# bmwoolf/mini_parallel

Measured on AMD Instinct MI355X. Metric: GCUPS (billion cell updates/s) on 150bp reads, 1/2/4/8 MI355X; bit-exact scores, higher is better.
Workload: dtype f16

## Files before the change

mini_parallel_amd/csrc/msw_device.h:

```cpp
#pragma once
#include "msw_kernels.h"

#include <type_traits>

namespace msw {

typedef unsigned short u16x2 __attribute__((ext_vector_type(2)));
typedef _Float16 f16x2 __attribute__((ext_vector_type(2)));

__device__ __forceinline__ uint32_t pk_satsub(uint32_t a, uint32_t b) {
    return __builtin_bit_cast(uint32_t, __builtin_elementwise_sub_sat(
        __builtin_bit_cast(u16x2, a), __builtin_bit_cast(u16x2, b)));
}
__device__ __forceinline__ uint32_t pk_add(uint32_t a, uint32_t b) {
    return __builtin_bit_cast(uint32_t, __builtin_bit_cast(u16x2, a) + __builtin_bit_cast(u16x2, b));
}
__device__ __forceinline__ uint32_t pk_min(uint32_t a, uint32_t b) {
    return __builtin_bit_cast(uint32_t, __builtin_elementwise_min(
        __builtin_bit_cast(u16x2, a), __builtin_bit_cast(u16x2, b)));
}
__device__ __forceinline__ uint32_t pk_max(uint32_t a, uint32_t b) {
    return __builtin_bit_cast(uint32_t, __builtin_elementwise_max(
        __builtin_bit_cast(u16x2, a), __builtin_bit_cast(u16x2, b)));
}
__device__ __forceinline__ uint32_t pk_max3(uint32_t a, uint32_t b, uint32_t c) {
    f16x2 x = __builtin_bit_cast(f16x2, a), y = __builtin_bit_cast(f16x2, b),
          z = __builtin_bit_cast(f16x2, c);
    return __builtin_bit_cast(uint32_t,
                              __builtin_elementwise_maximum(x, __builtin_elementwise_maximum(y, z)));
}
__device__ __forceinline__ uint32_t hadd(uint32_t a, uint32_t b) {
    return __builtin_bit_cast(uint32_t, __builtin_bit_cast(f16x2, a) + __builtin_bit_cast(f16x2, b));
}
__device__ __forceinline__ uint32_t hadd_clamp(uint32_t a, uint32_t b) {
    const f16x2 z = {(_Float16)0.0f, (_Float16)0.0f}, one = {(_Float16)1.0f, (_Float16)1.0f};
    const f16x2 v = __builtin_bit_cast(f16x2, a) + __builtin_bit_cast(f16x2, b);
    return __builtin_bit_cast(uint32_t, __builtin_elementwise_min(__builtin_elementwise_max(v, z), one));
}
__device__ __forceinline__ uint32_t hmax(uint32_t a, uint32_t b) {
    return __builtin_bit_cast(uint32_t, __builtin_elementwise_maximum(__builtin_bit_cast(f16x2, a),
                                                                      __builtin_bit_cast(f16x2, b)));
}
__device__ __forceinline__ uint32_t f16_to_score(uint32_t bits) {
    return (uint32_t)((float)__builtin_bit_cast(_Float16, (unsigned short)bits) * 2048.0f);
}

__device__ __forceinline__ uint32_t track_max3(uint32_t best, uint32_t a, uint32_t b) {
    uint32_t d;
    asm("v_pk_maximum3_f16 %0, %1, %2, %3" : "=v"(d) : "v"(best), "v"(a), "v"(b));
    return d;
}

__device__ __forceinline__ uint32_t shr1_group(uint32_t src, uint32_t top_mask) {
    return (uint32_t)__builtin_amdgcn_update_dpp(0, (int)src, 0x138, 0xF, 0xF, true) & top_mask;
}

__device__ __forceinline__ uint32_t add_nc(uint32_t a, uint32_t b) { return a + b; }

__device__ __forceinline__ uint32_t hi_to_lo_own_lo_to_hi(uint32_t own, uint32_t dpp) {
    return __builtin_amdgcn_alignbit(own, dpp, 16);
}

struct PairMeta {
    uint32_t pa, pb;
    uint32_t oa, ob;
    bool va, vb;
    int ma, mb, na, nb;
    int64_t sa, sb;
};

#ifndef MSW_PROBE_NO_WIN
#define MSW_PROBE_NO_WIN 0
#endif
#ifndef MSW_PROBE_NO_READ
#define MSW_PROBE_NO_READ 0
#endif
#ifndef MSW_PROBE_CONST_LEN
#define MSW_PROBE_CONST_LEN 0
#endif

template <bool SPLIT, bool GEN>
__device__ __forceinline__ PairMeta load_meta(const SwParams& p, int g, uint32_t block, bool active) {
    PairMeta q;
    const uint32_t slot_a = block * pairs_per_wave(SPLIT, p.groups) + (SPLIT ? g : 2u * g);
    const uint32_t slot_b = SPLIT ? slot_a : slot_a + 1;
    const uint32_t last = p.n_slots - 1;
    const uint32_t sa = min(slot_a, last), sb = min(slot_b, last);
    q.va = active && slot_a < p.n_slots;
    q.vb = active && slot_b < p.n_slots;
    q.pa = p.order ? p.order[sa] : p.slot_base + sa;
    q.pb = SPLIT ? q.pa : (p.order ? p.order[sb] : p.slot_base + sb);
    q.oa = p.out_by_slot ? p.out_slot_base + sa : q.pa;
    q.ob = p.out_by_slot ? p.out_slot_base + sb : q.pb;
    int ma, na, mb, nb;
    if (p.slot_lens) {
        const uint32_t la = p.slot_lens[p.out_slot_base + sa];
        const uint32_t lb = SPLIT ? la : p.slot_lens[p.out_slot_base + sb];
        ma = (int)(la & 0xFFFFu);
        na = (int)(la >> 16);
        mb = (int)(lb & 0xFFFFu);
        nb = (int)(lb >> 16);
    } else if (MSW_PROBE_CONST_LEN) {
        ma = mb = 150;
        na = nb = 300;
    } else {
        ma = p.read_len[q.pa];
        na = p.win_len[q.pa];
        mb = SPLIT ? ma : (int)p.read_len[q.pb];
        nb = SPLIT ? na : (int)p.win_len[q.pb];
    }
    q.ma = q.va ? ma : 0;
    q.mb = q.vb ? mb : 0;
    q.na = q.va ? na : 0;
    q.nb = q.vb ? nb : 0;
    if constexpr (GEN) {
        const int64_t sa = p.win_pos[q.pa];
        const int64_t sb = SPLIT ? sa : p.win_pos[q.pb];
        q.sa = q.na > 0 ? sa : 0;
        q.sb = q.nb > 0 ? sb : 0;
    }
    return q;
}

template <bool GEN>
__device__ __forceinline__ const uint8_t* win_row(const SwParams& p, uint32_t pair, int64_t pos) {
    if constexpr (GEN) return p.win_src + pos;
    else return p.wins + (uint64_t)pair * p.win_stride;
}

template <bool GEN>
__device__ __forceinline__ uint4 win_chunk(const uint8_t* row, int k) {
    const uint8_t* a = row + 16 * k;
    if constexpr (!GEN) {
        return *reinterpret_cast<const uint4*>(a);
    } else {
        const uint32_t b = (uint32_t)(reinterpret_cast<uintptr_t>(a) & 3u);
        const uint32_t* al = reinterpret_cast<const uint32_t*>(a - b);
        const uint32_t x0 = al[0], x1 = al[1], x2 = al[2], x3 = al[3], x4 = al[4];
        return make_uint4(__builtin_amdgcn_alignbyte(x1, x0, b), __builtin_amdgcn_alignbyte(x2, x1, b),
                          __builtin_amdgcn_alignbyte(x3, x2, b), __builtin_amdgcn_alignbyte(x4, x3, b));
    }
}

template <bool GEN>
__device__ __forceinline__ int win_last(const SwParams& p, int n) {
    if constexpr (GEN) return max(n, 1) - 1;
    else return (int)p.win_stride - 1;
}

__device__ __forceinline__ int wave_max_i32(int v) {
#pragma unroll
    for (int off = 32; off > 0; off >>= 1) v = max(v, __shfl_xor(v, off, 64));
    return v;
}

__device__ __forceinline__ int wave_max_nonneg(int v) {
    v = max(v, __builtin_amdgcn_update_dpp(0, v, 0x111, 0xF, 0xF, true));
    v = max(v, __builtin_amdgcn_update_dpp(0, v, 0x112, 0xF, 0xF, true));
    v = max(v, __builtin_amdgcn_update_dpp(0, v, 0x114, 0xF, 0xF, true));
    v = max(v, __builtin_amdgcn_update_dpp(0, v, 0x118, 0xF, 0xF, true));
    v = max(v, __builtin_amdgcn_update_dpp(0, v, 0x142, 0xA, 0xF, false));
    v = max(v, __builtin_amdgcn_update_dpp(0, v, 0x143, 0xC, 0xF, false));
    return __builtin_amdgcn_readlane(v, 63);
}

__device__ __forceinline__ uint32_t wcode(uint32_t byte, bool valid, uint32_t shift) {
    return valid ? (byte << shift) : kWinSentinel;
}

template <bool SPLIT, bool GEN>
__device__ __forceinline__ void stage_window(const SwParams& p, const PairMeta& q, uint32_t* stream,
                                             int steps, int lg, int G, bool active) {
    if (!active) return;
    const uint8_t* wa = win_row<GEN>(p, q.pa, q.sa);
    const uint8_t* wb = win_row<GEN>(p, q.pb, q.sb);
    const uint32_t sh = p.code_shift;
    const int last = win_last<GEN>(p, q.na), last_b = win_last<GEN>(p, q.nb);
    for (int k = lg; k < kLead; k += G) stream[k] = kWinSentinel2;
    const int nch = (steps + 15) >> 4;
    if (p.win_vec) {
        const int loadable = (int)(p.win_stride >> 4);
        const int top_a = GEN ? max((q.na + 15) / 16 - 1, 0) : 0, top_b = GEN ? max((q.nb + 15) / 16 - 1, 0) : 0;
        for (int k0 = 0; k0 < nch; k0 += 2 * G) {
            uint4 va[2], vb[2];
            uint32_t prev[2];
#pragma unroll
            for (int u = 0; u < 2; ++u) {
                const int k = k0 + u * G + lg;
                if constexpr (GEN) {
                    va[u] = win_chunk<true>(wa, min(k, top_a));
                    if constexpr (SPLIT) prev[u] = wa[min(max(16 * k - 1, 0), last)];
                    else vb[u] = win_chunk<true>(wb, min(k, top_b));
                } else {
                    const bool ld = k < nch && k < loadable && !MSW_PROBE_NO_WIN;
                    va[u] = ld ? *reinterpret_cast<const uint4*>(wa + 16 * k) : make_uint4(0, 0, 0, 0);
                    if constexpr (SPLIT) {
                        prev[u] = wa[min(max(16 * k - 1, 0), last)];
                    } else {
                        vb[u] = ld ? *reinterpret_cast<const uint4*>(wb + 16 * k) : make_uint4(0, 0, 0, 0);
                    }
                }
            }
#pragma unroll
            for (int u = 0; u < 2; ++u) {
                const int k = k0 + u * G + lg;
                if (k < nch) {
                    const uint32_t xa[4] = {va[u].x, va[u].y, va[u].z, va[u].w};
                    uint32_t xb[4] = {0u, 0u, 0u, 0u};
                    if constexpr (!SPLIT) { xb[0] = vb[u].x; xb[1] = vb[u].y; xb[2] = vb[u].z; xb[3] = vb[u].w; }
                    uint4* dst = reinterpret_cast<uint4*>(stream + kLead + 16 * k);
                    uint32_t carry = 0u;
                    if constexpr (SPLIT) carry = prev[u] & 0xFFu;
#pragma unroll
                    for (int d = 0; d < 4; ++d) {
                        uint32_t w4[4];
#pragma unroll
                        for (int e = 0; e < 4; ++e) {
                            const int c = 16 * k + 4 * d + e;
                            const uint32_t ba = (xa[d] >> (8 * e)) & 0xFFu;
                            if constexpr (SPLIT) {
                                w4[e] = wcode(ba, c < q.na, sh) | (wcode(carry, c >= 1 && c - 1 < q.na, sh) << 16);
                                carry = ba;
                            } else {
                                const uint32_t bb = (xb[d] >> (8 * e)) & 0xFFu;
                                w4[e] = wcode(ba, c < q.na, sh) | (wcode(bb, c < q.nb, sh) << 16);
                            }
                        }
                        dst[d] = make_uint4(w4[0], w4[1], w4[2], w4[3]);
                    }
                }
            }
        }
    } else {
        for (int c0 = 0; c0 < steps; c0 += 4 * G) {
            uint32_t ba[4], bb[4];
#pragma unroll
            for (int u = 0; u < 4; ++u) {
                const int c = c0 + u * G + lg;
                ba[u] = wa[min(c, last)];
                bb[u] = SPLIT ? wa[min(max(c - 1, 0), last)] : wb[min(c, GEN ? last_b : last)];
            }
#pragma unroll
            for (int u = 0; u < 4; ++u) {
                const int c = c0 + u * G + lg;
                const bool vb = SPLIT ? (c >= 1 && c - 1 < q.na) : (c < q.nb);
                if (c < steps) stream[kLead + c] = wcode(ba[u], c < q.na, sh) | (wcode(bb[u], vb, sh) << 16);
            }
        }
    }
}

template <int KR, bool SPLIT>
__device__ __forceinline__ void load_read_bytes(const SwParams& p, uint32_t pa, uint32_t pb, int lg,
                                                uint32_t (&ba)[KR], uint32_t (&bb)[KR]) {
    const uint8_t* ra = p.reads + (uint64_t)pa * p.read_stride;
    const uint8_t* rb = p.reads + (uint64_t)pb * p.read_stride;
    const int last = (int)p.read_stride - 1;
#pragma unroll
    for (int r = 0; r < KR; ++r) {
        const int ia = SPLIT ? lg * 2 * KR + r : lg * KR + r;
        const int ib = SPLIT ? ia + KR : ia;
#if MSW_PROBE_NO_READ
        ba[r] = (uint32_t)(ia + pa) & 3u;
        bb[r] = (uint32_t)(ib + pb) & 3u;
        (void)ra; (void)rb; (void)last;
#else
        ba[r] = ra[min(ia, last)];
        bb[r] = rb[min(ib, last)];
#endif
    }
}

template <int KR, bool SPLIT>
__device__ __forceinline__ void read_codes(const SwParams& p, const PairMeta& q, int lg, const uint32_t (&ba)[KR],
                                           const uint32_t (&bb)[KR], uint32_t (&rc)[KR]) {
#pragma unroll
    for (int r = 0; r < KR; ++r) {
        const int ia = SPLIT ? lg * 2 * KR + r : lg * KR + r;
        const int ib = SPLIT ? ia + KR : ia;
        const uint32_t ca = ia < q.ma ? (ba[r] << p.code_shift) : kReadSentinel;
        const uint32_t cb = ib < q.mb ? (bb[r] << p.code_shift) : kReadSentinel;
        rc[r] = ca | (cb << 16);
    }
}

__device__ __forceinline__ uint32_t group_pk_max(uint32_t v, int lg, int G) {
    const int lane = threadIdx.x;
#pragma unroll
    for (int off = 1; off < 16; off <<= 1) {
        const uint32_t o = (uint32_t)__shfl((int)v, lane + off, 64);
        v = lg + off < G ? pk_max(v, o) : v;
    }
    return v;
}

__device__ __forceinline__ uint64_t group_max_u64(uint64_t v, int lg, int G) {
    const int lane = threadIdx.x;
#pragma unroll
    for (int off = 1; off < 16; off <<= 1) {
        const uint64_t o = __shfl(v, lane + off, 64);
        v = (lg + off < G && o > v) ? o : v;
    }
    return v;
}

__device__ __forceinline__ void store_score(const SwParams& p, bool valid, uint32_t pair, uint32_t s) {
    if (valid) p.score[pair] = (int32_t)s;
}

__device__ __forceinline__ void store_hit(const SwParams& p, bool valid, uint32_t pair, uint64_t key,
                                          uint32_t bias, bool f16) {
    if (!valid) return;
    const uint32_t s = f16 ? f16_to_score((uint32_t)(key >> 32)) : (uint32_t)(key >> 32) - bias;
    p.score[pair] = (int32_t)s;
    if (p.end_i) {
        const uint32_t lo = (uint32_t)key;
        p.end_i[pair] = s ? (int16_t)(0xFFFFu - (lo >> 16)) : (int16_t)-1;
        p.end_j[pair] = s ? (int16_t)(0xFFFFu - (lo & 0xFFFFu)) : (int16_t)-1;
    }
}

template <int KR, bool SPLIT>
__device__ __forceinline__ void finish_coords(const SwParams& p, const PairMeta& q, int lg, int G,
                                              const uint32_t (&key_a)[KR], const uint32_t (&key_b)[KR],
                                              uint32_t bias, bool f16) {
    uint64_t ga = 0, gb = 0;
#pragma unroll
    for (int r = 0; r < KR; ++r) {
        const uint32_t ia = SPLIT ? (uint32_t)(lg * 2 * KR + r) : (uint32_t)(lg * KR + r);
        const uint32_t ib = SPLIT ? ia + KR : ia;
        const uint64_t ka = ((uint64_t)(key_a[r] >> 16) << 32) | ((uint64_t)(0xFFFFu - ia) << 16) |
                            (key_a[r] & 0xFFFFu);
        const uint64_t kb = ((uint64_t)(key_b[r] >> 16) << 32) | ((uint64_t)(0xFFFFu - ib) << 16) |
                            (key_b[r] & 0xFFFFu);
        ga = ka > ga ? ka : ga;
        gb = kb > gb ? kb : gb;
    }
    if constexpr (SPLIT) {
        ga = gb > ga ? gb : ga;
        ga = group_max_u64(ga, lg, G);
        if (lg == 0) store_hit(p, q.va, q.oa, ga, bias, f16);
    } else {
        ga = group_max_u64(ga, lg, G);
        gb = group_max_u64(gb, lg, G);
        if (lg == 0) {
            store_hit(p, q.va, q.oa, ga, bias, f16);
            store_hit(p, q.vb, q.ob, gb, bias, f16);
        }
    }
}

template <bool SPLIT>
__device__ __forceinline__ void finish_score(const SwParams& p, const PairMeta& q, int lg, int G,
                                             uint32_t best, uint32_t bias, bool f16) {
    best = group_pk_max(best, lg, G);
    if (lg == 0) {
        auto val = [&](uint32_t h) { return f16 ? f16_to_score(h) : h - bias; };
        if constexpr (SPLIT) {
            store_score(p, q.va, q.oa, val(max(best & 0xFFFFu, best >> 16)));
        } else {
            store_score(p, q.va, q.oa, val(best & 0xFFFFu));
            store_score(p, q.vb, q.ob, val(best >> 16));
        }
    }
}

template <bool SPLIT>
__device__ __forceinline__ uint32_t from_above(uint32_t own_bottom, uint32_t top_mask) {
    const uint32_t d = shr1_group(own_bottom, top_mask);
    if constexpr (SPLIT) return hi_to_lo_own_lo_to_hi(own_bottom, d);
    else return d;
}

__device__ __forceinline__ uint32_t base_class(uint32_t b) { return ((b >> 1) ^ (b >> 2)) & 3u; }

__device__ __forceinline__ bool is_acgt(uint32_t b) {
    const uint32_t o = b - 0x41u;
    return o < 20u && ((0x80045u >> o) & 1u);
}

__device__ __forceinline__ bool code_ok(uint32_t v, uint32_t shift) {
    return (v & kWinSentinel) || is_acgt(v >> shift);
}

__device__ __forceinline__ uint32_t win_selector(uint32_t word, uint32_t shift) {
    const uint32_t lo = word & 0xFFFFu, hi = word >> 16;
    const uint32_t sl = (lo & kWinSentinel) ? 12u : base_class(lo >> shift);
    const uint32_t sh = (hi & kWinSentinel) ? 12u : 4u + base_class(hi >> shift);
    return 12u | (sl << 8) | (12u << 16) | (sh << 24);
}

__device__ __forceinline__ uint32_t row_table(uint32_t v, uint32_t shift, uint32_t mis4, uint32_t match_hi) {
    const uint32_t b = v >> shift;
    if ((v & kReadSentinel) || !is_acgt(b)) return mis4;
    const uint32_t sh = 8u * base_class(b);
    return (mis4 & ~(0xFFu << sh)) | (match_hi << sh);
}

__device__ __forceinline__ bool to_fast_path(uint32_t* stream, int words, int lg, int G, bool active,
                                             uint32_t shift, bool allowed) {
    if (!allowed) return false;
    bool ok = true;
    for (int k = lg; active && k < words; k += G) {
        const uint32_t w = stream[k];
        ok = ok && code_ok(w & 0xFFFFu, shift) && code_ok(w >> 16, shift);
    }
    if (__builtin_amdgcn_ballot_w64(!ok) != 0) return false;
    for (int k = lg; active && k < words; k += G) stream[k] = win_selector(stream[k], shift);
    __syncthreads();
    return true;
}

__device__ __forceinline__ uint32_t class4(uint32_t x) { return ((x >> 1) ^ (x >> 2)) & 0x03030303u; }
__device__ __forceinline__ uint32_t canon4(uint32_t cl) { return __builtin_amdgcn_perm(0u, 0x54474341u, cl); }
__device__ __forceinline__ uint32_t byte_mask(int rem) {
    return rem >= 4 ? ~0u : (rem <= 0 ? 0u : ~0u >> (32 - 8 * rem));
}

constexpr int kRound = 2;
struct WinRound {
    uint4 a[kRound], b[kRound];
    uint32_t prev[kRound];
};

template <bool SPLIT, bool GEN>
__device__ __forceinline__ void load_round(const SwParams& p, const PairMeta& q, int k0, int lg, int G,
                                           WinRound& w) {
    const uint8_t* wa = win_row<GEN>(p, q.pa, q.sa);
    const uint8_t* wb = win_row<GEN>(p, q.pb, q.sb);
    const int stream_top = (int)((p.lds_stride - kLead) >> 4);
    const int top = (GEN ? stream_top : min((int)(p.win_stride >> 4), stream_top)) - 1;
    const int top_a = max(min(top, ((q.na + 15) >> 4) - 1), 0);
    const int top_b = max(min(top, ((q.nb + 15) >> 4) - 1), 0);
    const int last = win_last<GEN>(p, q.na);
#pragma unroll
    for (int u = 0; u < kRound; ++u) {
        const int k = k0 + u * G + lg;
#if MSW_PROBE_NO_WIN
        w.a[u] = w.b[u] = make_uint4(0x03020100u + min(k, top), 0x01000302u, 0x02010003u, 0x00030201u ^ q.pa);
        w.prev[u] = 0;
        (void)wa; (void)wb; (void)last; (void)top_a; (void)top_b;
#else
        w.a[u] = win_chunk<GEN>(wa, min(k, top_a));
        if constexpr (SPLIT) w.prev[u] = wa[min(max(16 * k - 1, 0), last)];
        else w.b[u] = win_chunk<GEN>(wb, min(k, top_b));
#endif
    }
}

template <bool SPLIT>
__device__ __forceinline__ uint32_t sel_round(const PairMeta& q, uint32_t* stream, int k0, int nch, int lg, int G,
                                              const WinRound& w) {
    uint32_t bad = 0u;
#pragma unroll
    for (int u = 0; u < kRound; ++u) {
        const int k = k0 + u * G + lg;
        if (k < nch) {
            const uint32_t xa[4] = {w.a[u].x, w.a[u].y, w.a[u].z, w.a[u].w};
            uint32_t xb[4] = {0u, 0u, 0u, 0u};
            if constexpr (!SPLIT) { xb[0] = w.b[u].x; xb[1] = w.b[u].y; xb[2] = w.b[u].z; xb[3] = w.b[u].w; }
            uint32_t carry = SPLIT ? (w.prev[u] & 0xFFu) : 0u;
            uint4* dst = reinterpret_cast<uint4*>(stream + kLead + 16 * k);
#pragma unroll
            for (int d = 0; d < 4; ++d) {
                const int c0 = 16 * k + 4 * d;
                const uint32_t x_a = xa[d];
                const uint32_t ma = byte_mask(q.na - c0);
                uint32_t x_b, mb;
                if constexpr (SPLIT) {
                    x_b = (x_a << 8) | carry;
                    carry = x_a >> 24;
                    mb = byte_mask(q.na + 1 - c0) & (c0 == 0 ? ~0xFFu : ~0u);
                } else {
                    x_b = xb[d];
                    mb = byte_mask(q.nb - c0);
                }
                const uint32_t ca = class4(x_a), cb = class4(x_b);
                bad |= ((canon4(ca) ^ x_a) & ma) | ((canon4(cb) ^ x_b) & mb);
                const uint32_t sa = (ca & ma) | (0x0C0C0C0Cu & ~ma);
                const uint32_t sb = ((cb | 0x04040404u) & mb) | (0x0C0C0C0Cu & ~mb);
                uint32_t o[4];
#pragma unroll
                for (int e = 0; e < 4; ++e)
                    o[e] = __builtin_amdgcn_perm(sb, sa, 0x000C000Cu | (uint32_t)e << 8 | (uint32_t)(4 + e) << 24) |
                           0x000C000Cu;
                dst[d] = make_uint4(o[0], o[1], o[2], o[3]);
            }
        }
    }
    return bad;
}

constexpr bool explicit_sched(bool affine, bool coords) { return !affine || coords; }
constexpr int step_unroll(bool , bool coords) { return coords ? 2 : 4; }
constexpr int perm_lead(bool affine, bool coords) { return !affine && !coords ? 2 : 0; }

template <int KR, bool AFFINE, bool COORDS, bool SPLIT, bool GEN = false>
__device__ __forceinline__ bool sw_body(const SwParams& p, uint32_t block, uint32_t* lds, uint64_t& t_loop) {
    const int lane = threadIdx.x;
    const int G = (int)p.group_lanes;
    const int g_raw = lane / G;
    const bool active = g_raw < (int)p.groups;
    const int g = active ? g_raw : 0;
    const int lg = active ? lane - g_raw * G : 0;
    uint32_t top_mask = lg == 0 ? 0u : ~0u;
    asm volatile("" : "+v"(top_mask));
    const PairMeta q = load_meta<SPLIT, GEN>(p, g, block, active);
    uint32_t rb_a[KR], rb_b[KR];
    load_read_bytes<KR, SPLIT>(p, q.pa, q.pb, lg, rb_a, rb_b);
    const bool try_fast = p.f16_ok && p.win_vec;
    WinRound w0;
    if (try_fast) load_round<SPLIT, GEN>(p, q, 0, lg, G, w0);
    const int skew = SPLIT ? 2 * (G - 1) + 1 : G - 1;
    constexpr int kUnroll = (!SPLIT && explicit_sched(AFFINE, COORDS)) ? 4 : step_unroll(AFFINE, COORDS);
    const int steps = (wave_max_nonneg(max(q.na, q.nb)) + skew + kUnroll - 1) & ~(kUnroll - 1);
    uint32_t* stream = lds + g * p.lds_stride;
    uint32_t rc[KR];
    read_codes<KR, SPLIT>(p, q, lg, rb_a, rb_b, rc);
    bool fast;
    if (try_fast) {
        const int nch = (int)((p.lds_stride - kLead) >> 4);
        uint32_t bad = 0u;
        if (active) {
            for (int k = lg; k < kLead; k += G) stream[k] = 0x0C0C0C0Cu;
            bad = sel_round<SPLIT>(q, stream, 0, nch, lg, G, w0);
            for (int k0 = kRound * G; k0 < nch; k0 += kRound * G) {
                WinRound w;
                load_round<SPLIT, GEN>(p, q, k0, lg, G, w);
                bad |= sel_round<SPLIT>(q, stream, k0, nch, lg, G, w);
            }
        }
        fast = __builtin_amdgcn_ballot_w64(bad != 0u) == 0;
        if (!fast) stage_window<SPLIT, GEN>(p, q, stream, steps, lg, G, active);
    } else {
        stage_window<SPLIT, GEN>(p, q, stream, steps, lg, G, active);
        __syncthreads();
        fast = to_fast_path(stream, kLead + steps, lg, G, active, p.code_shift, p.f16_ok != 0);
    }
    __syncthreads();

    uint32_t E[KR], GK[AFFINE ? KR : 1];
    uint32_t key_a[COORDS ? KR : 1], key_b[COORDS ? KR : 1];
    uint32_t best = 0u;
    const uint32_t* wp = stream + (kLead - (SPLIT ? 2 * lg : lg));
    const uint32_t nj_lane = (uint32_t)(0xFFFF + (SPLIT ? 2 * lg : lg));
    const uint32_t lds_wp = (uint32_t)(uintptr_t)wp;

    auto run = [&](auto f16_tag) __attribute__((always_inline)) {
        constexpr bool F16 = decltype(f16_tag)::value;
        const uint32_t match2 = p.match2, delta2 = p.delta2, ext2 = p.gap2, oe2 = p.open_ext2;
        const uint32_t bias2 = (AFFINE && !F16) ? p.bias2 : 0u;
        const uint32_t kmatch2 = add_nc(bias2, match2);
        const uint32_t og2 = oe2 - bias2;
        const uint32_t nge = p.f16_ngap2, noe = p.f16_noe2;
        uint32_t tab_lo[F16 ? KR : 1], tab_hi[F16 ? KR : 1];
        if constexpr (F16) {
            const uint32_t mis4 = (p.f16_hi >> 8) * 0x01010101u, match_hi = p.f16_hi & 0xFFu;
#pragma unroll
            for (int r = 0; r < KR; ++r) {
                tab_lo[r] = row_table(rc[r] & 0xFFFFu, p.code_shift, mis4, match_hi);
                tab_hi[r] = row_table(rc[r] >> 16, p.code_shift, mis4, match_hi);
            }
        }
        auto sub = [&](int r, uint32_t w) __attribute__((always_inline)) -> uint32_t {
            if constexpr (F16) return __builtin_amdgcn_perm(tab_hi[r], tab_lo[r], w);
            else return pk_min(rc[r] ^ w, delta2);
        };
#pragma unroll
        for (int r = 0; r < KR; ++r) {
            E[r] = bias2;
            if constexpr (AFFINE) GK[r] = bias2;
            if constexpr (COORDS) { key_a[r] = 0u; key_b[r] = 0u; }
        }
        uint32_t f_bot = bias2, h_bot = bias2;

        uint32_t t1a[KR], t1b[KR];
        using P0 = std::integral_constant<int, 0>;
        using P1 = std::integral_constant<int, 1>;
        if constexpr (F16 && !SPLIT && explicit_sched(AFFINE, COORDS)) {
#define MSW_SB __builtin_amdgcn_sched_barrier(0)
            {
                const uint32_t w0 = wp[0];
#pragma unroll
                for (int r = 0; r < KR; ++r) t1a[r] = sub(r, w0);
            }
            uint32_t an0 = sub(0, wp[1]);
            uint32_t hpend = 0u, hkm2 = 0u;
            uint32_t hu = shr1_group(h_bot, top_mask);
            uint32_t fu = AFFINE ? shr1_group(f_bot, top_mask) : 0u;
            auto sstep = [&](int t, uint32_t w1, uint32_t w2, const uint32_t (&t1)[KR], uint32_t (&t1n)[KR],
                             auto parity) __attribute__((always_inline)) {
                constexpr int kParity = decltype(parity)::value;
                uint32_t up = 0u, g_up = 0u, e_next = 0u, fsub = 0u;
                if constexpr (AFFINE) {
                    fsub = hadd(fu, nge);
                    MSW_SB;
                    g_up = hadd_clamp(hu, noe);
                    MSW_SB;
                    const uint32_t el = hadd(E[0], nge);
                    MSW_SB;
                    t1n[0] = hadd(hu, an0);
                    MSW_SB;
                    e_next = hmax(el, GK[0]);
                    MSW_SB;
                } else {
                    up = hadd_clamp(hu, nge);
                    MSW_SB;
                    t1n[0] = hadd(hu, an0);
                    MSW_SB;
                }
                uint32_t nja = 0u;
                if constexpr (COORDS) {
                    nja = (nj_lane - (uint32_t)t) & 0xFFFFu;
                    MSW_SB;
                } else if constexpr (KR & 1) {
                    if constexpr (kParity == 0) {
                        best = track_max3(best, hpend, h_bot);
                        MSW_SB;
                    } else {
                        hpend = h_bot;
                    }
                } else {
                    best = track_max3(best, hkm2, h_bot);
                    MSW_SB;
                }
                uint32_t hh[KR];
                uint32_t ka = 0u, kb = 0u;
                auto key_form = [&](int r) __attribute__((always_inline)) {
                    ka = (hh[r] << 16) | nja;
                    MSW_SB;
                    kb = (hh[r] & 0xFFFF0000u) | nja;
                    MSW_SB;
                };
                auto key_fold = [&](int r) __attribute__((always_inline)) {
                    key_a[r] = max(key_a[r], ka);
                    MSW_SB;
                    key_b[r] = max(key_b[r], kb);
                    MSW_SB;
                };
#pragma unroll
                for (int r = 0; r < KR; ++r) {
                    const bool last = r + 1 == KR;
                    uint32_t h, a = 0u;
                    if constexpr (AFFINE) {
                        const uint32_t e = e_next;
                        const uint32_t F = hmax(fsub, g_up);
                        MSW_SB;
                        uint32_t el = 0u;
                        if (!last) {
                            el = hadd(E[r + 1], nge);
                            MSW_SB;
                            a = sub(r + 1, w1);
                        } else {
                            an0 = sub(0, w2);
                        }
                        MSW_SB;
                        h = pk_max3(t1[r], e, F);
                        MSW_SB;
                        hh[r] = h;
                        E[r] = e;
                        if (!last) fsub = hadd(F, nge);
                        else fu = shr1_group(F, top_mask);
                        MSW_SB;
                        if (!last) {
                            e_next = hmax(el, GK[r + 1]);
                            MSW_SB;
                        }
                        if constexpr (COORDS) {
                            if (r > 0) key_form(r - 1);
                        }
                        g_up = GK[r] = hadd_clamp(h, noe);
                        MSW_SB;
                    } else {
                        h = pk_max3(t1[r], E[r], up);
                        MSW_SB;
                        hh[r] = h;
                        if (!last) a = sub(r + 1, w1);
                        else an0 = sub(0, w2);
                        MSW_SB;
                        if constexpr (COORDS) {
                            if (r > 0) key_form(r - 1);
                        }
                        up = E[r] = hadd_clamp(h, nge);
                        MSW_SB;
                    }
                    if (!last) {
                        t1n[r + 1] = hadd(h, a);
                        MSW_SB;
                    }
                    if constexpr (COORDS) {
                        if (r > 0) key_fold(r - 1);
                    } else if (r >= 2 && (r & 1) == 0) {
                        best = track_max3(best, hh[r - 2], hh[r - 1]);
                        MSW_SB;
                    }
                }
                if constexpr (COORDS) {
                    key_form(KR - 1);
                    key_fold(KR - 1);
                }
                h_bot = hh[KR - 1];
                if constexpr (!COORDS && (KR & 1) == 0) hkm2 = hh[KR - 2];
                hu = shr1_group(h_bot, top_mask);
                MSW_SB;
            };
            uint2 wa = make_uint2(wp[1], wp[2]);
            uint2 wb;
            asm volatile("ds_read2_b32 %0, %1 offset0:3 offset1:4" : "=v"(wb) : "v"(lds_wp));
            for (int t = 0; t < steps; t += 4) {
                const uint32_t base = lds_wp + 4u * (uint32_t)t;
                asm volatile("s_waitcnt lgkmcnt(0)" : "+v"(wb));
                sstep(t, wa.x, wa.y, t1a, t1b, P0{});
                sstep(t + 1, wa.y, wb.x, t1b, t1a, P1{});
                asm volatile("ds_read2_b32 %0, %1 offset0:5 offset1:6" : "=v"(wa) : "v"(base));
                sstep(t + 2, wb.x, wb.y, t1a, t1b, P0{});
                asm volatile("s_waitcnt lgkmcnt(0)" : "+v"(wa));
                sstep(t + 3, wb.y, wa.x, t1b, t1a, P1{});
                asm volatile("ds_read2_b32 %0, %1 offset0:7 offset1:8" : "=v"(wb) : "v"(base));
            }
            asm volatile("s_waitcnt lgkmcnt(0)" : "+v"(wb));
            if constexpr (!COORDS) best = track_max3(best, (KR & 1) ? hpend : hkm2, h_bot);
#undef MSW_SB
            return;
        }
        {
            const uint32_t w0 = wp[0];
#pragma unroll
            for (int r = 0; r < KR; ++r) {
                const uint32_t a = sub(r, w0);
                t1a[r] = F16 ? a : (AFFINE ? kmatch2 - a : pk_satsub(match2, a));
            }
        }
        uint32_t hpend = 0u;
        auto step = [&](int t, uint32_t w, const uint32_t (&t1)[KR], uint32_t (&t1n)[KR], auto parity)
                        __attribute__((always_inline)) {
            constexpr int kParity = decltype(parity)::value;
            const uint32_t h_up = from_above<SPLIT>(h_bot - bias2, top_mask);
            uint32_t up;
            uint32_t g_up;
            if constexpr (F16) {
                if constexpr (AFFINE) {
                    up = from_above<SPLIT>(f_bot, top_mask);
                    g_up = hadd_clamp(h_up, noe);
                } else {
                    up = hadd_clamp(h_up, nge);
                    g_up = 0u;
                }
            } else if constexpr (AFFINE) {
                up = add_nc(from_above<SPLIT>(f_bot - bias2, top_mask), bias2);
                g_up = add_nc(pk_satsub(h_up, og2), bias2);
            } else {
                up = pk_satsub(h_up, ext2);
                g_up = 0u;
            }
            constexpr int kPermLead = F16 ? perm_lead(AFFINE, COORDS) : 0;
            uint32_t a_n[KR];
#pragma unroll
            for (int r = 0; r < KR; ++r)
                if (!kPermLead || r < kPermLead) a_n[r] = sub(r, w);
            if constexpr (F16) t1n[0] = hadd(h_up, a_n[0]);
            else t1n[0] = AFFINE ? add_nc(h_up, kmatch2) - a_n[0] : pk_satsub(add_nc(h_up, kmatch2), a_n[0]);
            const uint32_t nj_a = (nj_lane - (uint32_t)t) & 0xFFFFu;
            const uint32_t nj_b = SPLIT ? ((nj_lane + 1u - (uint32_t)t) & 0xFFFFu) : nj_a;
            uint32_t hprev = 0u;
#pragma unroll
            for (int r = 0; r < KR; ++r) {
                uint32_t h;
                if constexpr (F16) {
                    if (kPermLead && r + kPermLead < KR) a_n[r + kPermLead] = sub(r + kPermLead, w);
                    if constexpr (AFFINE) {
                        const uint32_t e = hmax(hadd(E[r], nge), GK[r]);
                        up = hmax(hadd(up, nge), g_up);
                        h = pk_max3(t1[r], e, up);
                        E[r] = e;
                        g_up = GK[r] = hadd_clamp(h, noe);
                    } else {
                        h = pk_max3(t1[r], E[r], up);
                        up = E[r] = hadd_clamp(h, nge);
                    }
                    if (r + 1 < KR) t1n[r + 1] = hadd(h, a_n[r + 1]);
                } else if constexpr (AFFINE) {
                    const uint32_t e = pk_max(E[r] - ext2, GK[r]);
                    up = pk_max(up - ext2, g_up);
                    h = pk_max3(t1[r], e, up);
                    E[r] = e;
                    g_up = GK[r] = add_nc(pk_satsub(h, oe2), bias2);
                    if (r + 1 < KR) t1n[r + 1] = add_nc(h, match2) - a_n[r + 1];
                } else {
                    h = pk_max3(t1[r], E[r], up);
                    up = E[r] = pk_satsub(h, ext2);
                    if (r + 1 < KR) t1n[r + 1] = pk_satsub(add_nc(h, match2), a_n[r + 1]);
                }
                if (r + 1 == KR) h_bot = h;
                if constexpr (COORDS) {
                    key_a[r] = max(key_a[r], (h << 16) | nj_a);
                    key_b[r] = max(key_b[r], (h & 0xFFFF0000u) | nj_b);
                } else {
                    if (r & 1) {
                        best = track_max3(best, hprev, h);
                    } else if (r + 1 == KR) {
                        if constexpr (kParity == 0) hpend = h;
                        else best = track_max3(best, hpend, h);
                    }
                    hprev = h;
                }
                if constexpr (kPermLead > 0) __builtin_amdgcn_sched_barrier(0);
            }
            if constexpr (AFFINE) f_bot = up;
        };
        if constexpr (kUnroll == 4) {
            uint2 wa = make_uint2(wp[1], wp[2]);
            uint2 wb;
            asm volatile("ds_read2_b32 %0, %1 offset0:3 offset1:4" : "=v"(wb) : "v"(lds_wp));
            for (int t = 0; t < steps; t += 4) {
                const uint32_t base = lds_wp + 4u * (uint32_t)t;
                step(t, wa.x, t1a, t1b, P0{});
                step(t + 1, wa.y, t1b, t1a, P1{});
                asm volatile("ds_read2_b32 %0, %1 offset0:5 offset1:6" : "=v"(wa) : "v"(base));
                asm volatile("s_waitcnt lgkmcnt(1)" : "+v"(wb));
                step(t + 2, wb.x, t1a, t1b, P0{});
                step(t + 3, wb.y, t1b, t1a, P1{});
                asm volatile("ds_read2_b32 %0, %1 offset0:7 offset1:8" : "=v"(wb) : "v"(base));
                asm volatile("s_waitcnt lgkmcnt(1)" : "+v"(wa));
            }
            asm volatile("s_waitcnt lgkmcnt(0)" : "+v"(wb));
        } else {
            uint32_t w1 = wp[1], w2 = wp[2];
            uint2 wn;
            asm volatile("ds_read2_b32 %0, %1 offset0:3 offset1:4" : "=v"(wn) : "v"(lds_wp));
            for (int t = 0; t < steps; t += 2) {
                step(t, w1, t1a, t1b, P0{});
                step(t + 1, w2, t1b, t1a, P1{});
                asm volatile("s_waitcnt lgkmcnt(0)" : "+v"(wn));
                w1 = wn.x;
                w2 = wn.y;
                asm volatile("ds_read2_b32 %0, %1 offset0:3 offset1:4"
                             : "=v"(wn) : "v"(lds_wp + 4u * (uint32_t)(t + 2)));
            }
            asm volatile("s_waitcnt lgkmcnt(0)" : "+v"(wn));
        }
    };
    if (p.trace) t_loop = __builtin_amdgcn_s_memrealtime();
    if (fast) run(std::true_type{});
    else run(std::false_type{});

    const uint32_t bias = fast ? 0u : (p.bias2 & 0xFFFFu) * (AFFINE ? 1u : 0u);
    if constexpr (COORDS) finish_coords<KR, SPLIT>(p, q, lg, G, key_a, key_b, bias, fast);
    else finish_score<SPLIT>(p, q, lg, G, best, bias, fast);
    return fast;
}

struct WaveClock {
    uint64_t t0, c0;
};
__device__ __forceinline__ WaveClock trace_begin(const SwParams& p) {
    WaveClock w{0, 0};
    if (p.trace) {
        w.t0 = __builtin_amdgcn_s_memrealtime();
        w.c0 = __builtin_amdgcn_s_memtime();
    }
    return w;
}
__device__ __forceinline__ void trace_end(const SwParams& p, const WaveClock& w, bool fast, bool split,
                                          int kr, uint64_t t_loop) {
    if (!p.trace) return;
    const uint64_t t1 = __builtin_amdgcn_s_memrealtime();
    const uint64_t c1 = __builtin_amdgcn_s_memtime();
    if (threadIdx.x == 0) {
        const uint32_t hw_id = __builtin_amdgcn_s_getreg((4) | (0 << 6) | (31 << 11));
        const uint32_t xcc = __builtin_amdgcn_s_getreg((20) | (0 << 6) | (3 << 11));
        uint64_t* o = p.trace + 4ull * blockIdx.x;
        o[0] = w.t0;
        o[1] = t1;
        o[2] = (uint64_t)hw_id | ((uint64_t)xcc << 32) | ((uint64_t)fast << 40) | ((uint64_t)split << 41) |
               ((uint64_t)kr << 48);
        o[3] = ((c1 - w.c0) & 0xFFFFFFFFFFull) | ((t_loop - w.t0) << 40);
    }
}

template <uint32_t G>
__device__ __forceinline__ uint32_t xcd_block(uint32_t b, uint32_t nb) {
    constexpr uint32_t span = 8u * G;
    const uint32_t base = b - b % span;
    if (base + span > nb) return b;
    const uint32_t r = b - base;
    return base + (r % 8u) * G + r / 8u;
}

template <int KR, bool AFFINE, bool COORDS, bool SPLIT, bool GEN = false>
__global__ __launch_bounds__(64) void sw_kernel(SwParams p) {
    extern __shared__ __attribute__((aligned(16))) uint32_t lds[];
    const WaveClock wc = trace_begin(p);
    uint64_t t_loop = 0;
    const bool fast = sw_body<KR, AFFINE, COORDS, SPLIT, GEN>(p, blockIdx.x, lds, t_loop);
    trace_end(p, wc, fast, SPLIT, KR, t_loop);
}

template <int KRP, bool AFFINE, bool COORDS>
__global__ __launch_bounds__(64) void sw_mixed_kernel(SwParams p) {
    extern __shared__ __attribute__((aligned(16))) uint32_t lds[];
    const WaveClock wc = trace_begin(p);
    uint64_t t_loop = 0;
    if (blockIdx.x < p.pairs_blocks) {
        const bool fast = sw_body<KRP, AFFINE, COORDS, false>(p, blockIdx.x, lds, t_loop);
        trace_end(p, wc, fast, false, KRP, t_loop);
    } else {
        SwParams q = p;
        const uint32_t done = p.pairs_blocks * pairs_per_wave(false, p.groups);
        q.n_slots = p.n_slots - done;
        q.order = p.order ? p.order + done : nullptr;
        if (!p.order) q.slot_base = done;
        q.out_slot_base = p.out_slot_base + done;
        const bool fast = sw_body<(KRP + 1) / 2, AFFINE, COORDS, true>(q, blockIdx.x - p.pairs_blocks, lds,
                                                                      t_loop);
        trace_end(p, wc, fast, true, (KRP + 1) / 2, t_loop);
    }
}

template <int KR, bool AFFINE, bool COORDS>
__device__ __forceinline__ void multi_body(const SwParams& q, uint32_t blk, uint32_t* lds) {
    const WaveClock wc = trace_begin(q);
    uint64_t t_loop = 0;
    const bool fast = sw_body<KR, AFFINE, COORDS, false>(q, blk, lds, t_loop);
    trace_end(q, wc, fast, false, KR, t_loop);
}

template <bool AFFINE, bool COORDS, bool WIDE = false>
__global__ __launch_bounds__(64) void sw_multi_kernel(SwParams p, MultiTable t) {
    extern __shared__ __attribute__((aligned(16))) uint32_t lds[];
    const uint32_t lb = xcd_block<4>(blockIdx.x, gridDim.x);
    uint32_t b = 0;
    while (b + 1 < t.n_buckets && lb >= t.block_end[b]) ++b;
    const uint32_t blk = lb - (b ? t.block_end[b - 1] : 0u);
    SwParams q = p;
    q.order = p.order + t.slot_begin[b];
    q.out_slot_base = p.out_slot_base + t.slot_begin[b];
    q.n_slots = t.count[b];
    q.lds_stride = t.lds_stride[b];
    q.f16_ok = t.f16_ok[b];
    if constexpr (WIDE) {
        switch (t.kr[b]) {
            case 17: multi_body<17, AFFINE, COORDS>(q, blk, lds); break;
            case 18: multi_body<18, AFFINE, COORDS>(q, blk, lds); break;
            case 19: multi_body<19, AFFINE, COORDS>(q, blk, lds); break;
            case 20: multi_body<20, AFFINE, COORDS>(q, blk, lds); break;
            case 21: multi_body<21, AFFINE, COORDS>(q, blk, lds); break;
            case 22: multi_body<22, AFFINE, COORDS>(q, blk, lds); break;
            case 23: multi_body<23, AFFINE, COORDS>(q, blk, lds); break;
            default: multi_body<24, AFFINE, COORDS>(q, blk, lds); break;
        }
    } else {
        switch (t.kr[b]) {
            case 1: multi_body<1, AFFINE, COORDS>(q, blk, lds); break;
            case 2: multi_body<2, AFFINE, COORDS>(q, blk, lds); break;
            case 3: multi_body<3, AFFINE, COORDS>(q, blk, lds); break;
            case 4: multi_body<4, AFFINE, COORDS>(q, blk, lds); break;
            case 5: multi_body<5, AFFINE, COORDS>(q, blk, lds); break;
            case 6: multi_body<6, AFFINE, COORDS>(q, blk, lds); break;
            case 7: multi_body<7, AFFINE, COORDS>(q, blk, lds); break;
            case 8: multi_body<8, AFFINE, COORDS>(q, blk, lds); break;
            case 9: multi_body<9, AFFINE, COORDS>(q, blk, lds); break;
            case 10: multi_body<10, AFFINE, COORDS>(q, blk, lds); break;
            case 11: multi_body<11, AFFINE, COORDS>(q, blk, lds); break;
            case 12: multi_body<12, AFFINE, COORDS>(q, blk, lds); break;
            case 13: multi_body<13, AFFINE, COORDS>(q, blk, lds); break;
            case 14: multi_body<14, AFFINE, COORDS>(q, blk, lds); break;
            case 15: multi_body<15, AFFINE, COORDS>(q, blk, lds); break;
            default: multi_body<16, AFFINE, COORDS>(q, blk, lds); break;
        }
    }
}

}
```

Baseline: 10570.

## Specialize prologue for identity order, pin kernel args, simplify f16 row tables

Adds an identity-order specialization of load_meta that skips the order and slot_lens indirect loads when both are null, and hoists metadata masking after the read and window loads are issued so memory latency overlaps. It pins all kernel arguments into SGPRs with an empty asm, and computes f16 substitution tables directly from raw read bytes with a branchless XOR trick instead of going through read_codes. Window chunk clamping by length is dropped on the non-planned, non-generated path. The aim is a shorter per-wave prologue, at the cost of more code paths and possible out-of-range window chunk reads when clamping is skipped.

```diff
diff --git a/mini_parallel_amd/csrc/msw_device.h b/mini_parallel_amd/csrc/msw_device.h
--- a/mini_parallel_amd/csrc/msw_device.h
+++ b/mini_parallel_amd/csrc/msw_device.h
@@ -79,7 +79,28 @@
 #define MSW_PROBE_CONST_LEN 0
 #endif
 
-template <bool SPLIT, bool GEN>
+__device__ __forceinline__ void pin_args(const SwParams& p) {
+    asm volatile("" ::"s"(p.reads), "s"(p.wins), "s"(p.read_len), "s"(p.win_len), "s"(p.order), "s"(p.slot_lens),
+                 "s"(p.read_stride), "s"(p.win_stride), "s"(p.n_slots), "s"(p.lds_stride), "s"(p.code_shift),
+                 "s"(p.win_vec), "s"(p.slot_base), "s"(p.group_lanes), "s"(p.groups), "s"(p.f16_ok), "s"(p.f16_hi),
+                 "s"(p.f16_ngap2), "s"(p.out_by_slot), "s"(p.out_slot_base), "s"(p.score), "s"(p.match2),
+                 "s"(p.delta2), "s"(p.gap2), "s"(p.open_ext2), "s"(p.bias2), "s"(p.f16_noe2), "s"(p.end_i),
+                 "s"(p.end_j));
+}
+
+template <bool GEN>
+__device__ __forceinline__ void mask_meta(PairMeta& q) {
+    q.ma = q.va ? q.ma : 0;
+    q.mb = q.vb ? q.mb : 0;
+    q.na = q.va ? q.na : 0;
+    q.nb = q.vb ? q.nb : 0;
+    if constexpr (GEN) {
+        q.sa = q.na > 0 ? q.sa : 0;
+        q.sb = q.nb > 0 ? q.sb : 0;
+    }
+}
+
+template <bool SPLIT, bool GEN, bool IDENT>
 __device__ __forceinline__ PairMeta load_meta(const SwParams& p, int g, uint32_t block, bool active) {
     PairMeta q;
     const uint32_t slot_a = block * pairs_per_wave(SPLIT, p.groups) + (SPLIT ? g : 2u * g);
@@ -88,36 +109,34 @@
     const uint32_t sa = min(slot_a, last), sb = min(slot_b, last);
     q.va = active && slot_a < p.n_slots;
     q.vb = active && slot_b < p.n_slots;
-    q.pa = p.order ? p.order[sa] : p.slot_base + sa;
-    q.pb = SPLIT ? q.pa : (p.order ? p.order[sb] : p.slot_base + sb);
+    if constexpr (IDENT) {
+        q.pa = p.slot_base + sa;
+        q.pb = SPLIT ? q.pa : p.slot_base + sb;
+    } else {
+        q.pa = p.order ? p.order[sa] : p.slot_base + sa;
+        q.pb = SPLIT ? q.pa : (p.order ? p.order[sb] : p.slot_base + sb);
+    }
     q.oa = p.out_by_slot ? p.out_slot_base + sa : q.pa;
     q.ob = p.out_by_slot ? p.out_slot_base + sb : q.pb;
-    int ma, na, mb, nb;
-    if (p.slot_lens) {
+    if (!IDENT && p.slot_lens) {
         const uint32_t la = p.slot_lens[p.out_slot_base + sa];
         const uint32_t lb = SPLIT ? la : p.slot_lens[p.out_slot_base + sb];
-        ma = (int)(la & 0xFFFFu);
-        na = (int)(la >> 16);
-        mb = (int)(lb & 0xFFFFu);
-        nb = (int)(lb >> 16);
+        q.ma = (int)(la & 0xFFFFu);
+        q.na = (int)(la >> 16);
+        q.mb = (int)(lb & 0xFFFFu);
+        q.nb = (int)(lb >> 16);
     } else if (MSW_PROBE_CONST_LEN) {
-        ma = mb = 150;
-        na = nb = 300;
+        q.ma = q.mb = 150;
+        q.na = q.nb = 300;
     } else {
-        ma = p.read_len[q.pa];
-        na = p.win_len[q.pa];
-        mb = SPLIT ? ma : (int)p.read_len[q.pb];
-        nb = SPLIT ? na : (int)p.win_len[q.pb];
-    }
-    q.ma = q.va ? ma : 0;
-    q.mb = q.vb ? mb : 0;
-    q.na = q.va ? na : 0;
-    q.nb = q.vb ? nb : 0;
+        q.ma = p.read_len[q.pa];
+        q.na = p.win_len[q.pa];
+        q.mb = SPLIT ? q.ma : (int)p.read_len[q.pb];
+        q.nb = SPLIT ? q.na : (int)p.win_len[q.pb];
+    }
     if constexpr (GEN) {
-        const int64_t sa = p.win_pos[q.pa];
-        const int64_t sb = SPLIT ? sa : p.win_pos[q.pb];
-        q.sa = q.na > 0 ? sa : 0;
-        q.sb = q.nb > 0 ? sb : 0;
+        q.sa = p.win_pos[q.pa];
+        q.sb = SPLIT ? q.sa : p.win_pos[q.pb];
     }
     return q;
 }
@@ -390,11 +409,10 @@
     return 12u | (sl << 8) | (12u << 16) | (sh << 24);
 }
 
-__device__ __forceinline__ uint32_t row_table(uint32_t v, uint32_t shift, uint32_t mis4, uint32_t match_hi) {
-    const uint32_t b = v >> shift;
-    if ((v & kReadSentinel) || !is_acgt(b)) return mis4;
-    const uint32_t sh = 8u * base_class(b);
-    return (mis4 & ~(0xFFu << sh)) | (match_hi << sh);
+__device__ __forceinline__ uint32_t row_table(uint32_t b, bool in_read, uint32_t mis4, uint32_t d) {
+    const uint32_t sh = ((b << 2) ^ (b << 1)) & 0x18u;
+    const bool hit = in_read && ((0x54474341u >> sh) & 0xFFu) == b;
+    return mis4 ^ ((hit ? d : 0u) << sh);
 }
 
 __device__ __forceinline__ bool to_fast_path(uint32_t* stream, int words, int lg, int G, bool active,
@@ -423,15 +441,15 @@
     uint32_t prev[kRound];
 };
 
-template <bool SPLIT, bool GEN>
+template <bool SPLIT, bool GEN, bool CLAMP>
 __device__ __forceinline__ void load_round(const SwParams& p, const PairMeta& q, int k0, int lg, int G,
                                            WinRound& w) {
     const uint8_t* wa = win_row<GEN>(p, q.pa, q.sa);
     const uint8_t* wb = win_row<GEN>(p, q.pb, q.sb);
     const int stream_top = (int)((p.lds_stride - kLead) >> 4);
-    const int top = (GEN ? stream_top : min((int)(p.win_stride >> 4), stream_top)) - 1;
-    const int top_a = max(min(top, ((q.na + 15) >> 4) - 1), 0);
-    const int top_b = max(min(top, ((q.nb + 15) >> 4) - 1), 0);
+    const int top = max((GEN ? stream_top : min((int)(p.win_stride >> 4), stream_top)) - 1, 0);
+    const int top_a = CLAMP ? max(min(top, ((q.na + 15) >> 4) - 1), 0) : top;
+    const int top_b = CLAMP ? max(min(top, ((q.nb + 15) >> 4) - 1), 0) : top;
     const int last = win_last<GEN>(p, q.na);
 #pragma unroll
     for (int u = 0; u < kRound; ++u) {
@@ -495,7 +513,7 @@
 constexpr int step_unroll(bool , bool coords) { return coords ? 2 : 4; }
 constexpr int perm_lead(bool affine, bool coords) { return !affine && !coords ? 2 : 0; }
 
-template <int KR, bool AFFINE, bool COORDS, bool SPLIT, bool GEN = false>
+template <int KR, bool AFFINE, bool COORDS, bool SPLIT, bool GEN = false, bool PLAN = false>
 __device__ __forceinline__ bool sw_body(const SwParams& p, uint32_t block, uint32_t* lds, uint64_t& t_loop) {
     const int lane = threadIdx.x;
     const int G = (int)p.group_lanes;
@@ -505,18 +523,25 @@
     const int lg = active ? lane - g_raw * G : 0;
     uint32_t top_mask = lg == 0 ? 0u : ~0u;
     asm volatile("" : "+v"(top_mask));
-    const PairMeta q = load_meta<SPLIT, GEN>(p, g, block, active);
+    constexpr bool kClamp = PLAN || GEN;
+    const bool try_fast = p.f16_ok && p.win_vec;
+    PairMeta q;
     uint32_t rb_a[KR], rb_b[KR];
-    load_read_bytes<KR, SPLIT>(p, q.pa, q.pb, lg, rb_a, rb_b);
-    const bool try_fast = p.f16_ok && p.win_vec;
     WinRound w0;
-    if (try_fast) load_round<SPLIT, GEN>(p, q, 0, lg, G, w0);
+    auto early = [&](auto ident) __attribute__((always_inline)) {
+        q = load_meta<SPLIT, GEN, decltype(ident)::value>(p, g, block, active);
+        load_read_bytes<KR, SPLIT>(p, q.pa, q.pb, lg, rb_a, rb_b);
+        if constexpr (kClamp) mask_meta<GEN>(q);
+        if (try_fast) load_round<SPLIT, GEN, kClamp>(p, q, 0, lg, G, w0);
+        asm volatile("");
+    };
+    if (!PLAN && __builtin_expect(!p.order && !p.slot_lens, 1)) early(std::true_type{});
+    else early(std::false_type{});
+    if constexpr (!kClamp) mask_meta<GEN>(q);
     const int skew = SPLIT ? 2 * (G - 1) + 1 : G - 1;
     constexpr int kUnroll = (!SPLIT && explicit_sched(AFFINE, COORDS)) ? 4 : step_unroll(AFFINE, COORDS);
     const int steps = (wave_max_nonneg(max(q.na, q.nb)) + skew + kUnroll - 1) & ~(kUnroll - 1);
     uint32_t* stream = lds + g * p.lds_stride;
-    uint32_t rc[KR];
-    read_codes<KR, SPLIT>(p, q, lg, rb_a, rb_b, rc);
     bool fast;
     if (try_fast) {
         const int nch = (int)((p.lds_stride - kLead) >> 4);
@@ -526,7 +551,7 @@
             bad = sel_round<SPLIT>(q, stream, 0, nch, lg, G, w0);
             for (int k0 = kRound * G; k0 < nch; k0 += kRound * G) {
                 WinRound w;
-                load_round<SPLIT, GEN>(p, q, k0, lg, G, w);
+                load_round<SPLIT, GEN, kClamp>(p, q, k0, lg, G, w);
                 bad |= sel_round<SPLIT>(q, stream, k0, nch, lg, G, w);
             }
         }
@@ -546,6 +571,8 @@
     const uint32_t nj_lane = (uint32_t)(0xFFFF + (SPLIT ? 2 * lg : lg));
     const uint32_t lds_wp = (uint32_t)(uintptr_t)wp;
 
+    int t_first = 0;
+    asm("" : "+s"(t_first));
     auto run = [&](auto f16_tag) __attribute__((always_inline)) {
         constexpr bool F16 = decltype(f16_tag)::value;
         const uint32_t match2 = p.match2, delta2 = p.delta2, ext2 = p.gap2, oe2 = p.open_ext2;
@@ -553,14 +580,18 @@
         const uint32_t kmatch2 = add_nc(bias2, match2);
         const uint32_t og2 = oe2 - bias2;
         const uint32_t nge = p.f16_ngap2, noe = p.f16_noe2;
-        uint32_t tab_lo[F16 ? KR : 1], tab_hi[F16 ? KR : 1];
+        uint32_t tab_lo[F16 ? KR : 1], tab_hi[F16 ? KR : 1], rc[F16 ? 1 : KR];
         if constexpr (F16) {
-            const uint32_t mis4 = (p.f16_hi >> 8) * 0x01010101u, match_hi = p.f16_hi & 0xFFu;
+            const uint32_t mis4 = (p.f16_hi >> 8) * 0x01010101u, d = (p.f16_hi ^ (p.f16_hi >> 8)) & 0xFFu;
 #pragma unroll
             for (int r = 0; r < KR; ++r) {
-                tab_lo[r] = row_table(rc[r] & 0xFFFFu, p.code_shift, mis4, match_hi);
-                tab_hi[r] = row_table(rc[r] >> 16, p.code_shift, mis4, match_hi);
-            }
+                const int ia = SPLIT ? lg * 2 * KR + r : lg * KR + r;
+                const int ib = SPLIT ? ia + KR : ia;
+                tab_lo[r] = row_table(rb_a[r], ia < q.ma, mis4, d);
+                tab_hi[r] = row_table(rb_b[r], ib < q.mb, mis4, d);
+            }
+        } else {
+            read_codes<KR, SPLIT>(p, q, lg, rb_a, rb_b, rc);
         }
         auto sub = [&](int r, uint32_t w) __attribute__((always_inline)) -> uint32_t {
             if constexpr (F16) return __builtin_amdgcn_perm(tab_hi[r], tab_lo[r], w);
@@ -707,7 +738,7 @@
             uint2 wa = make_uint2(wp[1], wp[2]);
             uint2 wb;
             asm volatile("ds_read2_b32 %0, %1 offset0:3 offset1:4" : "=v"(wb) : "v"(lds_wp));
-            for (int t = 0; t < steps; t += 4) {
+            for (int t = t_first; t < steps; t += 4) {
                 const uint32_t base = lds_wp + 4u * (uint32_t)t;
                 asm volatile("s_waitcnt lgkmcnt(0)" : "+v"(wb));
                 sstep(t, wa.x, wa.y, t1a, t1b, P0{});
@@ -812,7 +843,7 @@
             uint2 wa = make_uint2(wp[1], wp[2]);
             uint2 wb;
             asm volatile("ds_read2_b32 %0, %1 offset0:3 offset1:4" : "=v"(wb) : "v"(lds_wp));
-            for (int t = 0; t < steps; t += 4) {
+            for (int t = t_first; t < steps; t += 4) {
                 const uint32_t base = lds_wp + 4u * (uint32_t)t;
                 step(t, wa.x, t1a, t1b, P0{});
                 step(t + 1, wa.y, t1b, t1a, P1{});
@@ -828,7 +859,7 @@
             uint32_t w1 = wp[1], w2 = wp[2];
             uint2 wn;
             asm volatile("ds_read2_b32 %0, %1 offset0:3 offset1:4" : "=v"(wn) : "v"(lds_wp));
-            for (int t = 0; t < steps; t += 2) {
+            for (int t = t_first; t < steps; t += 2) {
                 step(t, w1, t1a, t1b, P0{});
                 step(t + 1, w2, t1b, t1a, P1{});
                 asm volatile("s_waitcnt lgkmcnt(0)" : "+v"(wn));
@@ -890,6 +921,7 @@
 template <int KR, bool AFFINE, bool COORDS, bool SPLIT, bool GEN = false>
 __global__ __launch_bounds__(64) void sw_kernel(SwParams p) {
     extern __shared__ __attribute__((aligned(16))) uint32_t lds[];
+    pin_args(p);
     const WaveClock wc = trace_begin(p);
     uint64_t t_loop = 0;
     const bool fast = sw_body<KR, AFFINE, COORDS, SPLIT, GEN>(p, blockIdx.x, lds, t_loop);
@@ -899,6 +931,7 @@
 template <int KRP, bool AFFINE, bool COORDS>
 __global__ __launch_bounds__(64) void sw_mixed_kernel(SwParams p) {
     extern __shared__ __attribute__((aligned(16))) uint32_t lds[];
+    pin_args(p);
     const WaveClock wc = trace_begin(p);
     uint64_t t_loop = 0;
     if (blockIdx.x < p.pairs_blocks) {
@@ -921,13 +954,14 @@
 __device__ __forceinline__ void multi_body(const SwParams& q, uint32_t blk, uint32_t* lds) {
     const WaveClock wc = trace_begin(q);
     uint64_t t_loop = 0;
-    const bool fast = sw_body<KR, AFFINE, COORDS, false>(q, blk, lds, t_loop);
+    const bool fast = sw_body<KR, AFFINE, COORDS, false, false, true>(q, blk, lds, t_loop);
     trace_end(q, wc, fast, false, KR, t_loop);
 }
 
 template <bool AFFINE, bool COORDS, bool WIDE = false>
 __global__ __launch_bounds__(64) void sw_multi_kernel(SwParams p, MultiTable t) {
     extern __shared__ __attribute__((aligned(16))) uint32_t lds[];
+    pin_args(p);
     const uint32_t lb = xcd_block<4>(blockIdx.x, gridDim.x);
     uint32_t b = 0;
     while (b + 1 < t.n_buckets && lb >= t.block_end[b]) ++b;
```

Measured after the change: 10850 (median of 6 runs). 2.6% higher.
